# alguoo314/JASPER

Hardware: AMD Instinct MI355X
Metric: assembly Mbp/s polished + Gk-mers/s counted, k=37 (higher is better)
Workload: dtype u64

## Files before the change

### jasper_amd/csrc/polish.hip

```cpp
#include "polish.hpp"
#include <algorithm>

namespace jk {

constexpr int SMAX = 384;

__device__ __forceinline__ void pyslice(int64_t len, int64_t a, int64_t b, int64_t &lo, int64_t &hi) {
    if (a < 0) { a += len; if (a < 0) a = 0; } else if (a > len) a = len;
    if (b < 0) { b += len; if (b < 0) b = 0; } else if (b > len) b = len;
    if (b < a) b = a;
    lo = a; hi = b;
}

__device__ __forceinline__ int64_t pyround(double x) { return (int64_t)rint(x); }

struct FrontEntry {
    uint32_t node;
    uint16_t tlen;
    uint8_t alive;
    uint8_t pad;
    uint8_t tail[72];
};
static_assert(sizeof(FrontEntry) == 80, "FrontEntry layout");

// ... 951 lines not shown
                    __builtin_amdgcn_s_sleep(4);
                } else {
                    back += 64;
                    if (spins > (1u << 24)) { a = ARRIVE_FAIL; break; }
                }
            }
        }
        if (a < 0 || a < lo || a - C->seg_lo >= C->len0) {
            if (lane == 0) { C->spec_fail = 1; C->ticks = wall_clock64() - t0; }
            publish_arrival(C->arrive, ARRIVE_FAIL);
            return;
        }
        if (!dirty) {
            const int64_t stop = C->last ? C->cls_n : C->stop_orig;
            const int64_t steps = a >= stop ? 0 : (stop - a + (k - 2)) / (k - 1);
            if (lane == 0) {
                C->took_shortcut = 1;
                C->lookups = 2ull * (uint64_t)steps;
                C->ticks = wall_clock64() - t0;
            }
            publish_arrival(C->arrive, C->last ? ARRIVE_END : a + steps * (k - 1));
            return;
        }
        start_i = a - C->seg_lo;
    }
    Walker w;
    w.T = T; w.k = P.k; w.step = P.step; w.lane = threadIdx.x; w.solid = P.solid;
    w.buf = C->buf; w.len = C->len; w.gs = C->gs; w.glen = C->glen; w.cap = C->cap;
    w.C = C; w.chunk_id = C->chunk; w.nrec = 0; w.naux = 0; w.seqno = 0; w.nedit = 0; w.pass = pass;
    w.status = PS_OK; w.nlook = 0; for (int q = 0; q < 12; ++q) w.tk[q] = 0;
    w.s_tbf = s_tbf; w.s_t1 = s_t1; w.s_t2 = s_t2; w.s_gkb = s_gkb; w.s_gka = s_gka;
    w.delta = 0; w.dirty_end = INT64_MIN / 2; w.glo = P.k;
    w.is_first = C->first != 0; w.is_last = C->last != 0; w.spec_fail = 0;
    w.cls = C->cls; w.cls_n = C->cls_n; w.seg_lo = C->seg_lo; w.stop_orig = C->stop_orig;
    w.pool = pool; w.bfs_slot = -1; w.bfs_nodes = nullptr; w.bfs_front = nullptr; w.bfs_patch = nullptr;
    const bool fix = P.fix && pass < P.passes;
    int64_t wrong = 0;
    long long arrive = ARRIVE_FAIL;
    w.walk(fix, start_i, wrong, arrive);
    w.release_scratch();
    if (threadIdx.x == 0) {
        C->ticks = wall_clock64() - t0;
        for (int q = 0; q < 12; ++q) C->tk[q] = w.tk[q];
        C->len = w.len; C->gs = w.gs; C->glen = w.glen;
        C->nrec = w.nrec; C->naux = w.naux; C->nedit = w.nedit; C->status = w.status; C->spec_fail = w.spec_fail;
        C->wrong = wrong;
        C->lookups = w.nlook;
    }
    publish_arrival(C->arrive, arrive);
}

constexpr int SC_THREADS = 256, SC_GROUP = 16, SC_TILE = SC_THREADS * SC_GROUP, SC_HALO = 4;

__global__ __launch_bounds__(256) void seg_init_kernel(SegDev *segs, int n_segs, const uint8_t *const *chunk_text) {
    struct __attribute__((packed, aligned(1))) V16 { uint32_t w[4]; };
    for (int s = blockIdx.y; s < n_segs; s += gridDim.y) {
        const SegDev S = segs[s];
        const uint8_t *src = chunk_text[S.chunk] + S.seg_lo;
        uint8_t *dst = S.buf + S.glen;
        const int64_t nblk = (S.len0 + 15) >> 4;
        for (int64_t blk = blockIdx.x * (int64_t)blockDim.x + threadIdx.x; blk < nblk; blk += (int64_t)gridDim.x * blockDim.x) {
            const int64_t q0 = blk << 4;
            if (q0 + 16 <= S.len0) *reinterpret_cast<V16 *>(dst + q0) = *reinterpret_cast<const V16 *>(src + q0);
            else for (int64_t q = q0; q < S.len0; ++q) dst[q] = src[q];
        }
    }
}

constexpr uint32_t STITCH_MAX_EDITS = 32;
__global__ __launch_bounds__(256) void seg_stitch_kernel(const SegDev *segs, int n_segs, uint8_t *const *chunk_out, uint8_t *const *cls_out,
                                                         uint8_t *const *flags) {
    struct __attribute__((packed, aligned(1))) V16 { uint32_t w[4]; };
    for (int s = blockIdx.y; s < n_segs; s += gridDim.y) {
        const SegDev S = segs[s];
        uint8_t *dst = chunk_out[S.chunk] + S.out_off;
        uint8_t *cdst = cls_out ? cls_out[S.chunk] + S.out_off : nullptr;
        uint8_t *fl = cls_out ? flags[S.chunk] : nullptr;
        const int64_t n = S.own_hi - S.own_lo;
        const bool all_dirty = S.nedit > STITCH_MAX_EDITS;
        const int64_t nblk = (n + 15) >> 4;
        for (int64_t blk = blockIdx.x * (int64_t)blockDim.x + threadIdx.x; blk < nblk; blk += (int64_t)gridDim.x * blockDim.x) {
            const int64_t q0 = blk << 4;
            const int64_t p0 = S.own_lo + q0;
            const bool full = q0 + 16 <= n;
            bool text_done = false, cls_done = !cdst;
            if (full && (p0 + 16 <= S.gs || p0 >= S.gs)) {
                *reinterpret_cast<V16 *>(dst + q0) = *reinterpret_cast<const V16 *>(S.buf + (p0 < S.gs ? p0 : p0 + S.glen));
                text_done = true;
            }
            if (full && cdst && !all_dirty) {
                int64_t lA = p0, lB = p0 + 15;
                bool uniform = true;
                for (int e = (int)S.nedit - 1; e >= 0; --e) {
                    const EditRec E = S.edits[e];
                    if (lA > E.a + E.plen) { const int64_t d = (int64_t)E.plen - E.oldlen; lA -= d; lB -= d; }
                    else if (lB < E.a - 1) { }
                    else { uniform = false; break; }
                }
                if (uniform && S.seg_lo + lB < S.cls_n) {
                    *reinterpret_cast<V16 *>(cdst + q0) = *reinterpret_cast<const V16 *>(S.cls + S.seg_lo + lA);
                    cls_done = true;
                }
            }
            if (text_done && cls_done) continue;
            const int64_t qe = q0 + 16 < n ? q0 + 16 : n;
            for (int64_t q = q0; q < qe; ++q) {
                const int64_t p = S.own_lo + q;
                if (!text_done) dst[q] = S.buf[p < S.gs ? p : p + S.glen];
                if (cls_done) continue;
                int64_t l = p;
                bool dirty = all_dirty;
                if (!dirty)
                    for (int e = (int)S.nedit - 1; e >= 0; --e) {
                        const EditRec E = S.edits[e];
                        if (l > E.a + E.plen) l -= (int64_t)E.plen - E.oldlen;
                        else if (l >= E.a - 1) { dirty = true; break; }
                    }
                if (dirty) {
                    fl[(S.out_off + q) >> 6] = 1;
                    cdst[q] = PC_OTHER;
                } else {
                    const int64_t old = S.seg_lo + l;
                    cdst[q] = old < S.cls_n ? S.cls[old] : (uint8_t)PC_OTHER;
                }
            }
        }
    }
}

__global__ __launch_bounds__(64) void seg_gather_kernel(const SegDev *segs, int n_segs, const int64_t *idx_base, const uint32_t *seq_base,
                                                        const uint32_t *rec_off, const uint32_t *aux_off, FixRec *out_recs, uint8_t *out_aux) {
    const int s = blockIdx.x;
    if (s >= n_segs) return;
    const SegDev S = segs[s];
    for (uint32_t r = threadIdx.x; r < S.nrec; r += blockDim.x) {
        FixRec f = S.recs[r];
        f.index += idx_base[s];
        f.seqno += seq_base[s];
        if (f.kind == 'x') f.aux_off += aux_off[s];
        out_recs[rec_off[s] + r] = f;
    }
    for (uint32_t q = threadIdx.x; q < S.naux; q += blockDim.x) out_aux[aux_off[s] + q] = S.aux[q];
}

__device__ __forceinline__ long long wave_scan_incl64(long long v) {
    const int lane = threadIdx.x & 63;
#pragma unroll
    for (int o = 1; o < 64; o <<= 1) { const long long u = __shfl_up(v, o); if (lane >= o) v += u; }
    return v;
}
__global__ __launch_bounds__(64) void seg_summary_kernel(SegDev *segs, const int32_t *first_seg, int n_chunks, int64_t *idx_base, uint32_t *seq_base,
                                                         uint32_t *rec_off, uint32_t *aux_off, ChunkSummary *out) {
    const int c = blockIdx.x;
    if (c >= n_chunks) return;
    const int lane = threadIdx.x;
    const int s0 = first_seg[c], s1 = first_seg[c + 1];
    long long newlen = 0, shift = 0, seqc = 0, recc = 0, auxc = 0, wrong = 0, lookups = 0;
    int bad = -1, spec = 0;
    for (int base = s0; base < s1; base += 64) {
        const int s = base + lane;
        const bool in = s < s1;
        long long d = 0, own = 0, nrec = 0, naux = 0, seg_lo = 0, own_hi = 0;
        if (in) {
            SegDev &S = segs[s];
            d = S.len - S.len0;
            own_hi = S.last ? S.len : S.own_hi0 + d;
            own = own_hi - S.own_lo;
            nrec = S.nrec; naux = S.naux; seg_lo = S.seg_lo;
            wrong += S.wrong; lookups += (long long)S.lookups;
            if (S.status != PS_OK && (bad < 0 || s < bad)) bad = s;
            if (S.spec_fail && S.status == PS_OK) spec = 1;
        }
        const long long i_own = wave_scan_incl64(own), i_d = wave_scan_incl64(d), i_rec = wave_scan_incl64(nrec), i_aux = wave_scan_incl64(naux);
        if (in) {
            SegDev &S = segs[s];
            S.own_hi = own_hi;
            S.out_off = newlen + i_own - own;
            idx_base[s] = seg_lo + shift + i_d - d;
            seq_base[s] = (uint32_t)(seqc + i_rec - nrec);
            rec_off[s] = (uint32_t)(recc + i_rec - nrec);
            aux_off[s] = (uint32_t)(auxc + i_aux - naux);
        }
        newlen += __shfl(i_own, 63); shift += __shfl(i_d, 63);
        seqc += __shfl(i_rec, 63); recc += __shfl(i_rec, 63); auxc += __shfl(i_aux, 63);
    }
    for (int o = 32; o > 0; o >>= 1) {
        wrong += __shfl_xor(wrong, o); lookups += __shfl_xor(lookups, o);
        const int b2 = __shfl_xor(bad, o);
        bad = bad < 0 ? b2 : (b2 < 0 ? bad : (b2 < bad ? b2 : bad));
        spec |= __shfl_xor(spec, o);
    }
    if (lane == 0) {
        ChunkSummary R;
        R.newlen = newlen; R.wrong = wrong; R.lookups = (uint64_t)lookups; R.nrec = (uint32_t)recc; R.naux = (uint32_t)auxc; R.bad_seg = bad; R.spec_fail = spec;
        out[c] = R;
    }
}
__global__ __launch_bounds__(64) void seg_offsets_kernel(const int32_t *first_seg, int n_chunks, uint32_t *rec_off, uint32_t *aux_off, const ChunkSummary *sum) {
    const int c = blockIdx.x;
    if (c >= n_chunks || c == 0) return;
    const int lane = threadIdx.x;
    unsigned long long rb = 0, ab = 0;
    for (int q = lane; q < c; q += 64) { rb += sum[q].nrec; ab += sum[q].naux; }
    for (int o = 32; o > 0; o >>= 1) { rb += __shfl_xor(rb, o); ab += __shfl_xor(ab, o); }
    for (int s = first_seg[c] + lane; s < first_seg[c + 1]; s += 64) { rec_off[s] += (uint32_t)rb; aux_off[s] += (uint32_t)ab; }
}

constexpr int SC_BACK = 64;
constexpr int SC_STRIDE = SC_TILE - SC_BACK;
__global__ __launch_bounds__(SC_THREADS) void scan_classify_batch_kernel(const ScanChunk *__restrict__ chunks, int n_chunks, TableDev T, uint32_t solid) {
    __shared__ uint32_t s_code[SC_THREADS + SC_HALO];
    __shared__ uint32_t s_inv[SC_THREADS + SC_HALO];
    __shared__ uint32_t s_cnt[SC_TILE];
    __shared__ uint8_t s_ok[SC_TILE];
    const int t = threadIdx.x;
    const int k = T.k;
    const u128 kmask = maskbits(2 * k);
    for (int ci = blockIdx.y; ci < n_chunks; ci += gridDim.y) {
        const ScanChunk C = chunks[ci];
        const uint8_t *__restrict__ text = C.text;
        const int64_t n = C.len;
        const int64_t nwin = n - k + 1;
        if (nwin <= 0) continue;
        const int64_t ntiles = (n + SC_STRIDE - 1) / SC_STRIDE;
        for (int64_t tile = blockIdx.x; tile < ntiles; tile += gridDim.x) {
            const int64_t origin = tile * SC_STRIDE - SC_BACK;
            uint32_t c, iv;
            stage16(text, origin + (int64_t)t * SC_GROUP, n, c, iv);
            s_code[t + SC_HALO] = c;
            s_inv[t + SC_HALO] = iv;
            if (t < SC_HALO) {
                uint32_t hc, hiv;
                stage16(text, origin - (int64_t)(SC_HALO - t) * SC_GROUP, n, hc, hiv);
                s_code[t] = hc;
                s_inv[t] = hiv;
            }
            __syncthreads();
            const uint32_t w4 = s_code[t], w3 = s_code[t + 1], w2 = s_code[t + 2], w1 = s_code[t + 3];
            const uint64_t ivprev = ((uint64_t)s_inv[t] << 48) | ((uint64_t)s_inv[t + 1] << 32) | ((uint64_t)s_inv[t + 2] << 16) |
                                    (uint64_t)s_inv[t + 3];
            u128 fwd = band(mk(((uint64_t)w4 << 32) | w3, ((uint64_t)w2 << 32) | w1), kmask);
            u128 rc = revcomp(fwd, k);
            int run = ivprev ? (int)__builtin_ctzll(ivprev) : 64;
            const int64_t e0 = origin + (int64_t)t * SC_GROUP;
#pragma unroll
            for (int j0 = 0; j0 < SC_GROUP; j0 += 4) {
                u128 hs[4];
                bool ok[4];
                ulonglong2 ent[4];
#pragma unroll
                for (int u = 0; u < 4; ++u) {
                    const int j = j0 + u;
                    const uint32_t cj = (c >> (30 - 2 * j)) & 3u;
                    const bool bad = (iv >> (15 - j)) & 1u;
                    fwd = band(bor(shl(fwd, 2), mk(0, cj)), kmask);
                    rc = bor(shr(rc, 2), shl(mk(0, 3u - cj), 2 * (k - 1)));
                    run = bad ? 0 : run + 1;
                    const int64_t e = e0 + j;
                    ok[u] = run >= k && e - k + 1 >= 0 && e < n;
                    hs[u] = mix(lt(rc, fwd) ? rc : fwd, T.B);
                    ent[u] = make_ulonglong2(0ull, 0ull);
                    if (ok[u]) ent[u] = *reinterpret_cast<const ulonglong2 *>(read_slots(T, hs[u]) + 2 * home_of(hs[u], T.B, T.s));
                }
#pragma unroll
                for (int u = 0; u < 4; ++u) {
                    s_cnt[t * SC_GROUP + j0 + u] = ok[u] ? clamp32(table_get_prefetched(T, hs[u], ent[u])) : 0u;
                    s_ok[t * SC_GROUP + j0 + u] = ok[u] ? 1 : 0;
                }
            }
            __syncthreads();
            if (t >= SC_BACK / SC_GROUP) {
                struct __attribute__((packed, aligned(1))) V16 { uint32_t w[4]; };
                V16 out;
                out.w[0] = out.w[1] = out.w[2] = out.w[3] = 0;
                const int64_t p0 = e0 - k + 1;
#pragma unroll
                for (int j = 0; j < SC_GROUP; ++j) {
                    const int64_t p = p0 + j;
                    const uint32_t me = s_cnt[t * SC_GROUP + j];
                    uint8_t cl;
                    if (!s_ok[t * SC_GROUP + j]) cl = PC_OTHER;
                    else if (me < solid) cl = PC_BAD;
                    else if (p > 0) {
                        const int64_t qe = (p - k > 0 ? p - k : 0) + k - 1;
                        const int qi = (int)(qe - origin);
                        cl = (!s_ok[qi] || 50ull * me < (unsigned long long)s_cnt[qi]) ? PC_OTHER : PC_CLEAN;
                    } else cl = PC_CLEAN;
                    out.w[j >> 2] |= (uint32_t)cl << (8 * (j & 3));
                }
                if (p0 >= 0 && p0 + SC_GROUP <= nwin) *reinterpret_cast<V16 *>(C.cls + p0) = out;
                else {
#pragma unroll
                    for (int j = 0; j < SC_GROUP; ++j) {
                        const int64_t p = p0 + j;
                        if (p >= 0 && p < nwin) C.cls[p] = (uint8_t)((out.w[j >> 2] >> (8 * (j & 3))) & 0xFFu);
                    }
                }
            }
            __syncthreads();
        }
    }
}

__global__ __launch_bounds__(256) void find_sync_batch_kernel(const ScanChunk *__restrict__ chunks, int n_chunks, int k) {
    struct __attribute__((packed, aligned(1))) V16 { uint32_t w[4]; };
    const int64_t W = 4ll * k;
    for (int ci = blockIdx.y; ci < n_chunks; ci += gridDim.y) {
        const ScanChunk C = chunks[ci];
        if (!C.want_sync) continue;
        const int64_t nwin = C.len - k + 1;
        const uint8_t *__restrict__ cls = C.cls;
        static_assert(PC_CLEAN == 0 && PC_BAD == 1 && PC_OTHER == 2, "the block test below looks at bit 0 of the class bytes");
        const int64_t nblk = (nwin + 15) >> 4;
        for (int64_t blk = blockIdx.x * (int64_t)blockDim.x + threadIdx.x; blk < nblk; blk += (int64_t)gridDim.x * blockDim.x) {
            const int64_t p0 = blk << 4;
            uint32_t w[4];
            if (p0 + 16 <= nwin) {
                const V16 v = *reinterpret_cast<const V16 *>(cls + p0);
                w[0] = v.w[0]; w[1] = v.w[1]; w[2] = v.w[2]; w[3] = v.w[3];
                if (!((w[0] | w[1] | w[2] | w[3]) & 0x01010101u)) continue;
            }
            const int64_t pe = p0 + 16 < nwin ? p0 + 16 : nwin;
            for (int64_t p = p0; p < pe; ++p) {
                if (p < W || p + k - 1 > nwin) continue;
                if (cls[p] != PC_BAD || cls[p - 1] != PC_CLEAN) continue;
                uint32_t diff = 0;
                {
                    int64_t q = p + 1;
                    const int64_t qe = p + k - 1;
                    for (; q + 16 <= qe; q += 16) {
                        const V16 v = *reinterpret_cast<const V16 *>(cls + q);
                        diff |= (v.w[0] ^ 0x01010101u) | (v.w[1] ^ 0x01010101u) | (v.w[2] ^ 0x01010101u) | (v.w[3] ^ 0x01010101u);
                    }
                    for (; q < qe; ++q) diff |= (uint32_t)(cls[q] ^ (uint8_t)PC_BAD);
                    q = p - W;
                    const int64_t qf = p - 1;
                    for (; q + 16 <= qf; q += 16) {
                        const V16 v = *reinterpret_cast<const V16 *>(cls + q);
                        diff |= v.w[0] | v.w[1] | v.w[2] | v.w[3];
                    }
                    for (; q < qf; ++q) diff |= (uint32_t)cls[q];
                }
                if (diff) continue;
                const unsigned int idx = atomicAdd(C.cand_count, 1u);
                if (idx < C.cand_cap) C.cand[idx] = ((int64_t)ci << 40) | p;
            }
        }
    }
}

__global__ __launch_bounds__(256) void rescan_batch_kernel(const ScanChunk *__restrict__ chunks, int n_chunks, TableDev T, uint32_t solid) {
    __shared__ uint32_t s_cnt[4][128];
    __shared__ uint8_t s_valid[4][128];
    __shared__ uint8_t s_text[4][256];
    const int wave = threadIdx.x >> 6, lane = threadIdx.x & 63;
    const int k = T.k;
    for (int ci = blockIdx.y; ci < n_chunks; ci += gridDim.y) {
        const ScanChunk C = chunks[ci];
        const int64_t nwin = C.len - k + 1;
        if (nwin <= 0) continue;
        const int64_t ntile = (nwin + 63) >> 6, nflag = (C.len >> 6) + 1;
        const int64_t W = (int64_t)gridDim.x * 4;
        for (int64_t tile0 = (int64_t)blockIdx.x * 4 + wave; tile0 < ntile; tile0 += 64 * W) {
            uint8_t f = 0;
            {
                const int64_t tl = tile0 + (int64_t)lane * W;
                if (tl < ntile) {
                    f = C.flags[tl];
                    if (tl > 0) f |= C.flags[tl - 1];
                    if (tl + 1 < nflag) f |= C.flags[tl + 1];
                }
            }
            unsigned long long todo = __ballot(f != 0);
          while (todo) {
            const int64_t tile = tile0 + (int64_t)__builtin_ctzll(todo) * W;
            todo &= todo - 1ull;
            const int64_t base = tile * 64 - 64;
#pragma unroll
            for (int q = 0; q < 4; ++q) {
                const int64_t pos = base + (int64_t)lane * 4 + q;
                s_text[wave][lane * 4 + q] = (pos >= 0 && pos < C.len) ? C.text[pos] : (uint8_t)'N';
            }
            __builtin_amdgcn_fence(__ATOMIC_SEQ_CST, "workgroup");
            __builtin_amdgcn_wave_barrier();
#pragma unroll
            for (int r = 0; r < 2; ++r) {
                const int64_t p = base + r * 64 + lane;
                uint32_t cnt = 0;
                uint8_t valid = 0;
                if (p >= 0 && p < nwin) {
                    u128 fwd = mk(0, 0);
                    bool ok = true;
                    for (int j = 0; j < k; ++j) {
                        const int c = code(s_text[wave][r * 64 + lane + j]);
                        ok = ok && c >= 0;
                        fwd = bor(shl(fwd, 2), mk(0, (uint64_t)(c & 3)));
                    }
                    if (ok) {
                        cnt = clamp32(table_get(T, mix(canonical(fwd, k), T.B)));
                        valid = 1;
                    }
                }
                s_cnt[wave][r * 64 + lane] = cnt;
                s_valid[wave][r * 64 + lane] = valid;
            }
            __builtin_amdgcn_fence(__ATOMIC_SEQ_CST, "workgroup");
            __builtin_amdgcn_wave_barrier();
            const int64_t p = tile * 64 + lane;
            if (p < nwin) {
                const int me = 64 + lane;
                uint8_t c;
                if (!s_valid[wave][me]) c = PC_OTHER;
                else if (s_cnt[wave][me] < solid) c = PC_BAD;
                else if (p > 0) {
                    const int qi = p - k > 0 ? me - k : 64;
                    c = (!s_valid[wave][qi] || 50ull * s_cnt[wave][me] < (unsigned long long)s_cnt[wave][qi]) ? PC_OTHER : PC_CLEAN;
                } else c = PC_CLEAN;
                C.cls[p] = c;
            }
            __builtin_amdgcn_wave_barrier();
          }
        }
    }
}

__global__ __launch_bounds__(64) void find_clean_batch_kernel(const ScanChunk *__restrict__ chunks, int n_chunks, int k) {
    const int lane = threadIdx.x;
    for (int ci = blockIdx.y; ci < n_chunks; ci += gridDim.y) {
        const ScanChunk C = chunks[ci];
        const int64_t nwin = C.len - k + 1;
        for (uint32_t g = blockIdx.x; g < C.n_cells; g += gridDim.x) {
            int64_t p0 = (int64_t)g * CLEAN_CELL + CLEAN_CELL / 2;
            const int64_t cell_end = (int64_t)(g + 1) * CLEAN_CELL;
            int64_t cand = -1;
            for (int attempt = 0; attempt < 8; ++attempt) {
                if (p0 - 4ll * k < 0 || p0 + k > nwin || p0 + k > cell_end) break;
                int64_t last_bad = -1;
                for (int64_t q0 = p0 - 4ll * k; q0 < p0 + k; q0 += 64) {
                    const int64_t q = q0 + lane;
                    const bool nc = q < p0 + k && C.cls[q] != PC_CLEAN;
                    const uint64_t m = __ballot(nc);
                    if (m) last_bad = q0 + 63 - (int64_t)__builtin_clzll(m);
                }
                if (last_bad < 0) { cand = p0; break; }
                p0 = last_bad + 4ll * k + 1;
            }
            if (lane == 0) C.clean_cand[g] = cand;
        }
    }
}

static void launch_find_clean(const ScanChunk *d_chunks, int n_chunks, int k, hipStream_t stream) {
    const int gy = n_chunks < 1024 ? n_chunks : 1024;
    const int gx = std::max(1, 8192 / gy);
    hipLaunchKernelGGL(find_clean_batch_kernel, dim3(gx, gy), dim3(64), 0, stream, d_chunks, n_chunks, k);
}

void launch_rescan_batch(const TableDev &T, const ScanChunk *d_chunks, int n_chunks, int k, uint32_t solid, hipStream_t stream) {
    if (n_chunks <= 0) return;
    const int gy = n_chunks < 1024 ? n_chunks : 1024;
    const int gx = std::max(1, 4096 / gy);
    hipLaunchKernelGGL(rescan_batch_kernel, dim3(gx, gy), dim3(256), 0, stream, d_chunks, n_chunks, T, solid);
    hipLaunchKernelGGL(find_sync_batch_kernel, dim3(gx, gy), dim3(256), 0, stream, d_chunks, n_chunks, k);
    launch_find_clean(d_chunks, n_chunks, k, stream);
}

void launch_scan_batch(const TableDev &T, const ScanChunk *d_chunks, int n_chunks, int k, uint32_t solid, hipStream_t stream) {
    if (n_chunks <= 0) return;
    const int gy = n_chunks < 1024 ? n_chunks : 1024;
    const int gx = std::max(1, 4096 / gy);
    hipLaunchKernelGGL(scan_classify_batch_kernel, dim3(gx, gy), dim3(SC_THREADS), 0, stream, d_chunks, n_chunks, T, solid);
    hipLaunchKernelGGL(find_sync_batch_kernel, dim3(gx, gy), dim3(256), 0, stream, d_chunks, n_chunks, k);
    launch_find_clean(d_chunks, n_chunks, k, stream);
}

__global__ __launch_bounds__(256) void copy_chunks_kernel(uint8_t *const *__restrict__ chunk_ptr, uint8_t *__restrict__ pack, const int64_t *__restrict__ offs, int n,
                                                          int to_chunks) {
    for (int c = blockIdx.x; c < n; c += gridDim.x) {
        const int64_t len = offs[c + 1] - offs[c];
        uint8_t *a = chunk_ptr[c], *b = pack + offs[c];
        const uint8_t *src = to_chunks ? b : a;
        uint8_t *dst = to_chunks ? a : b;
        for (int64_t i = threadIdx.x; i < len; i += 256) dst[i] = src[i];
    }
}
void launch_copy_chunks(uint8_t *const *d_chunk_ptr, uint8_t *d_pack, const int64_t *d_offs, int n, bool to_chunks, hipStream_t stream) {
    if (n <= 0) return;
    hipLaunchKernelGGL(copy_chunks_kernel, dim3((unsigned)std::min(n, 256 * 16)), dim3(256), 0, stream, d_chunk_ptr, d_pack, d_offs, n, to_chunks ? 1 : 0);
}

void launch_seg_init(SegDev *d_segs, int n_segs, const uint8_t *const *d_chunk_text, hipStream_t stream) {
    if (n_segs <= 0) return;
    dim3 grid(n_segs >= 512 ? 4 : 64, n_segs < 4096 ? n_segs : 4096);
    hipLaunchKernelGGL(seg_init_kernel, grid, dim3(256), 0, stream, d_segs, n_segs, d_chunk_text);
}
void launch_seg_walk(const TableDev &T, SegDev *d_segs, int n_segs, PolishParams pp, int pass, ScratchPool pool, unsigned int *d_ticket,
                     hipStream_t stream) {
    if (n_segs <= 0) return;
    (void)hipMemsetAsync(d_ticket, 0, sizeof(unsigned int), stream);
    hipLaunchKernelGGL(seg_walk_kernel, dim3(n_segs), dim3(64), 0, stream, T, d_segs, n_segs, pp, pass, pool, d_ticket);
}
void launch_seg_summary(SegDev *d_segs, int n_segs, const int32_t *d_first_seg, int n_chunks, int64_t *idx_base, uint32_t *seq_base, uint32_t *rec_off,
                        uint32_t *aux_off, ChunkSummary *d_out, hipStream_t stream) {
    if (n_segs <= 0 || n_chunks <= 0) return;
    hipLaunchKernelGGL(seg_summary_kernel, dim3(n_chunks), dim3(64), 0, stream, d_segs, d_first_seg, n_chunks, idx_base, seq_base, rec_off, aux_off, d_out);
    hipLaunchKernelGGL(seg_offsets_kernel, dim3(n_chunks), dim3(64), 0, stream, d_first_seg, n_chunks, rec_off, aux_off, d_out);
}
void launch_seg_gather(const SegDev *d_segs, int n_segs, const int64_t *idx_base, const uint32_t *seq_base, const uint32_t *rec_off,
                       const uint32_t *aux_off, FixRec *out_recs, uint8_t *out_aux, hipStream_t stream) {
    if (n_segs <= 0) return;
    hipLaunchKernelGGL(seg_gather_kernel, dim3(n_segs), dim3(64), 0, stream, d_segs, n_segs, idx_base, seq_base, rec_off, aux_off, out_recs, out_aux);
}
void launch_seg_stitch(const SegDev *d_segs, int n_segs, uint8_t *const *d_chunk_out, uint8_t *const *d_cls_out, uint8_t *const *d_flags,
                       hipStream_t stream) {
    if (n_segs <= 0) return;
    dim3 grid(n_segs >= 2048 ? 2 : n_segs >= 512 ? 4 : 64, n_segs < 4096 ? n_segs : 4096);
    hipLaunchKernelGGL(seg_stitch_kernel, grid, dim3(256), 0, stream, d_segs, n_segs, d_chunk_out, d_cls_out, d_flags);
}

}
```

Measured before the change: 3057.

## Add specialized dense-table rescan kernel and fuse sync/clean mark kernels

```diff
diff --git a/jasper_amd/csrc/polish.hip b/jasper_amd/csrc/polish.hip
--- a/jasper_amd/csrc/polish.hip
+++ b/jasper_amd/csrc/polish.hip
@@ -1277,12 +1277,113 @@
     }
 }
 
-__global__ __launch_bounds__(256) void find_sync_batch_kernel(const ScanChunk *__restrict__ chunks, int n_chunks, int k) {
+template <int NW, int KFIX>
+struct DenseCore {
+    int k, sh;
+    int rsh;
+    uint32_t topmask, slotmask;
+    uint64_t lomask, himask, remmask;
+    uint32_t f[NW], r[NW];
+    __device__ __forceinline__ explicit DenseCore(const TableDev &T) {
+        k = KFIX ? KFIX : T.k;
+        const int B = 2 * k, topbits = B - 32 * (NW - 1), hb = B - 64;
+        sh = B - T.s;
+        rsh = topbits - 2;
+        topmask = topbits >= 32 ? ~0u : ((1u << topbits) - 1u);
+        slotmask = (uint32_t)T.mask;
+        lomask = B >= 64 ? ~0ull : ((1ull << B) - 1ull);
+        himask = NW > 2 ? (hb >= 64 ? ~0ull : ((1ull << hb) - 1ull)) : 0ull;
+        remmask = (1ull << sh) - 1ull;
+    }
+    __device__ __forceinline__ void start(u128 fwd0, u128 rc0) {
+        const uint32_t fw[4] = {(uint32_t)fwd0.lo, (uint32_t)(fwd0.lo >> 32), (uint32_t)fwd0.hi, (uint32_t)(fwd0.hi >> 32)};
+        const uint32_t rw[4] = {(uint32_t)rc0.lo, (uint32_t)(rc0.lo >> 32), (uint32_t)rc0.hi, (uint32_t)(rc0.hi >> 32)};
+#pragma unroll
+        for (int w = 0; w < NW; ++w) { f[w] = fw[w]; r[w] = rw[w]; }
+    }
+    __device__ __forceinline__ void roll(uint32_t cj) {
+#pragma unroll
+        for (int w = NW - 1; w > 0; --w) f[w] = __builtin_amdgcn_alignbit(f[w], f[w - 1], 30);
+        f[0] = (f[0] << 2) | cj;
+        f[NW - 1] &= topmask;
+#pragma unroll
+        for (int w = 0; w < NW - 1; ++w) r[w] = __builtin_amdgcn_alignbit(r[w + 1], r[w], 2);
+        r[NW - 1] = (r[NW - 1] >> 2) | ((cj ^ 3u) << rsh);
+    }
+    __device__ __forceinline__ void probe(uint32_t &home, uint64_t &want0) const {
+        static_assert(NW >= 1 && NW <= 3, "a narrow table holds no k-mer of more than three words: 2k - s <= 53");
+        uint32_t m[NW];
+        [[maybe_unused]] uint32_t d;
+        if constexpr (NW == 3) {
+            asm("v_sub_co_u32_e32 %3, vcc, %4, %7\n\tv_subb_co_u32_e32 %3, vcc, %5, %8, vcc\n\tv_subb_co_u32_e32 %3, vcc, %6, %9, vcc\n\t"
+                "v_cndmask_b32_e32 %0, %7, %4, vcc\n\tv_cndmask_b32_e32 %1, %8, %5, vcc\n\tv_cndmask_b32_e32 %2, %9, %6, vcc"
+                : "=&v"(m[0]), "=&v"(m[1]), "=&v"(m[2]), "=&v"(d) : "v"(r[0]), "v"(r[1]), "v"(r[2]), "v"(f[0]), "v"(f[1]), "v"(f[2]) : "vcc");
+        } else if constexpr (NW == 2) {
+            asm("v_sub_co_u32_e32 %2, vcc, %3, %5\n\tv_subb_co_u32_e32 %2, vcc, %4, %6, vcc\n\t"
+                "v_cndmask_b32_e32 %0, %5, %3, vcc\n\tv_cndmask_b32_e32 %1, %6, %4, vcc"
+                : "=&v"(m[0]), "=&v"(m[1]), "=&v"(d) : "v"(r[0]), "v"(r[1]), "v"(f[0]), "v"(f[1]) : "vcc");
+        } else {
+            m[0] = r[0] < f[0] ? r[0] : f[0];
+        }
+        uint64_t rem;
+        if constexpr (NW > 2) {
+            const uint64_t lo = mix64(((uint64_t)m[1] << 32) | m[0]);
+            const uint64_t hi = ((uint64_t)m[2] ^ rotr64(lo, 30)) & himask;
+            home = (uint32_t)((lo >> sh) | (hi << (64 - sh)));
+            rem = lo & remmask;
+        } else {
+            const int hh = k;
+            uint64_t v = m[0];
+            if constexpr (NW > 1) v |= (uint64_t)m[1] << 32;
+            v ^= v >> hh;
+            v = (v * JK_C1) & lomask;
+            v ^= v >> hh;
+            home = (uint32_t)(v >> sh);
+            rem = v & remmask;
+        }
+        want0 = OCC | (rem << OFFBITS);
+    }
+};
+static bool dense_core_serves(const TableDev &T) { return !T.ext && T.nshard <= 1 && T.s <= 32 && 2 * T.k - T.s >= 0 && 2 * T.k - T.s <= 63 - OFFBITS; }
+
+__device__ __forceinline__ ulonglong2 dense_load(const TableDev &T, uint32_t slotmask, uint32_t home, uint32_t off) {
+    return *reinterpret_cast<const ulonglong2 *>(T.slots + 2ull * (uint64_t)((home + off) & slotmask));
+}
+template <int U0, int U1, int N>
+__device__ __forceinline__ void dense_resolve(const ulonglong2 (&ent)[N], const uint64_t (&want0)[N], uint32_t off, uint32_t (&cnt)[N], uint32_t &pend) {
+#pragma unroll
+    for (int u = U0; u < U1; ++u) {
+        if ((pend >> u) & 1u) {
+            const bool hit = ent[u].x == want0[u] + off;
+            if (hit) cnt[u] = clamp32(ent[u].y);
+            if (hit || ent[u].x == 0ull) pend &= ~(1u << u);
+        }
+    }
+}
+template <int U0, int U1, int N>
+__device__ __forceinline__ void dense_issue(const TableDev &T, uint32_t slotmask, const uint32_t (&home)[N], uint32_t off, uint32_t pend, ulonglong2 (&ent)[N]) {
+#pragma unroll
+    for (int u = U0; u < U1; ++u)
+        if ((pend >> u) & 1u) ent[u] = dense_load(T, slotmask, home[u], off);
+}
+template <int N>
+__device__ __forceinline__ void dense_counts(const TableDev &T, uint32_t slotmask, const uint32_t (&home)[N], const uint64_t (&want0)[N], ulonglong2 (&ent)[N],
+                                             uint32_t pend, uint32_t (&cnt)[N]) {
+    constexpr int H = N / 2;
+#pragma unroll
+    for (int u = 0; u < N; ++u) cnt[u] = 0;
+    dense_resolve<0, H>(ent, want0, 0, cnt, pend);
+    dense_resolve<H, N>(ent, want0, 0, cnt, pend);
+    for (uint32_t off = 1; __ballot(pend != 0) && off < MAXPROBE; ++off) {
+        dense_issue<0, N>(T, slotmask, home, off, pend, ent);
+        dense_resolve<0, N>(ent, want0, off, cnt, pend);
+    }
+}
+
+__device__ __forceinline__ void find_sync_chunk(const ScanChunk &C, int ci, int k) {
     struct __attribute__((packed, aligned(1))) V16 { uint32_t w[4]; };
     const int64_t W = 4ll * k;
-    for (int ci = blockIdx.y; ci < n_chunks; ci += gridDim.y) {
-        const ScanChunk C = chunks[ci];
-        if (!C.want_sync) continue;
+    {
         const int64_t nwin = C.len - k + 1;
         const uint8_t *__restrict__ cls = C.cls;
         static_assert(PC_CLEAN == 0 && PC_BAD == 1 && PC_OTHER == 2, "the block test below looks at bit 0 of the class bytes");
@@ -1295,10 +1396,24 @@
                 w[0] = v.w[0]; w[1] = v.w[1]; w[2] = v.w[2]; w[3] = v.w[3];
                 if (!((w[0] | w[1] | w[2] | w[3]) & 0x01010101u)) continue;
             }
-            const int64_t pe = p0 + 16 < nwin ? p0 + 16 : nwin;
-            for (int64_t p = p0; p < pe; ++p) {
+            uint32_t startm = 0;
+            if (p0 + 16 <= nwin) {
+                uint32_t badm = 0, cleanm = 0;
+#pragma unroll
+                for (int j = 0; j < 16; ++j) {
+                    const uint32_t b = (w[j >> 2] >> (8 * (j & 3))) & 0xFFu;
+                    badm |= (b == PC_BAD ? 1u : 0u) << j;
+                    cleanm |= (b == PC_CLEAN ? 1u : 0u) << j;
+                }
+                startm = badm & ((cleanm << 1) | ((p0 > 0 && cls[p0 - 1] == PC_CLEAN) ? 1u : 0u));
+            } else {
+                for (int64_t p = p0 > 0 ? p0 : 1; p < nwin; ++p)
+                    if (cls[p] == PC_BAD && cls[p - 1] == PC_CLEAN) startm |= 1u << (int)(p - p0);
+            }
+            while (startm) {
+                const int64_t p = p0 + __builtin_ctz(startm);
+                startm &= startm - 1u;
                 if (p < W || p + k - 1 > nwin) continue;
-                if (cls[p] != PC_BAD || cls[p - 1] != PC_CLEAN) continue;
                 uint32_t diff = 0;
                 {
                     int64_t q = p + 1;
@@ -1399,12 +1514,98 @@
     }
 }
 
-__global__ __launch_bounds__(64) void find_clean_batch_kernel(const ScanChunk *__restrict__ chunks, int n_chunks, int k) {
-    const int lane = threadIdx.x;
+template <int NW, int KFIX>
+__global__ __launch_bounds__(256) void rescan_core_kernel(const ScanChunk *__restrict__ chunks, int n_chunks, TableDev T, uint32_t solid) {
+    constexpr int PADW = 4, TEXTW = 12;
+    __shared__ uint32_t s_cnt[4][128];
+    __shared__ uint8_t s_valid[4][128];
+    __shared__ uint32_t s_cw[4][PADW + TEXTW], s_iw[4][PADW + TEXTW];
+    const int wave = threadIdx.x >> 6, lane = threadIdx.x & 63;
+    DenseCore<NW, KFIX> K(T);
+    const int k = K.k;
+    const u128 kmask = maskbits(2 * k);
+    const uint64_t kbits = k >= 64 ? ~0ull : ((1ull << k) - 1ull);
+    if (lane < PADW) { s_cw[wave][lane] = 0; s_iw[wave][lane] = 0; }
     for (int ci = blockIdx.y; ci < n_chunks; ci += gridDim.y) {
         const ScanChunk C = chunks[ci];
         const int64_t nwin = C.len - k + 1;
-        for (uint32_t g = blockIdx.x; g < C.n_cells; g += gridDim.x) {
+        if (nwin <= 0) continue;
+        const int64_t ntile = (nwin + 63) >> 6, nflag = (C.len >> 6) + 1;
+        const int64_t W = (int64_t)gridDim.x * 4;
+        for (int64_t tile0 = (int64_t)blockIdx.x * 4 + wave; tile0 < ntile; tile0 += 64 * W) {
+            uint8_t f = 0;
+            {
+                const int64_t tl = tile0 + (int64_t)lane * W;
+                if (tl < ntile) {
+                    f = C.flags[tl];
+                    if (tl > 0) f |= C.flags[tl - 1];
+                    if (tl + 1 < nflag) f |= C.flags[tl + 1];
+                }
+            }
+            unsigned long long todo = __ballot(f != 0);
+          while (todo) {
+            const int64_t tile = tile0 + (int64_t)__builtin_ctzll(todo) * W;
+            todo &= todo - 1ull;
+            const int64_t base = tile * 64 - 64;
+            if (lane < TEXTW) {
+                uint32_t c, iv;
+                stage16(C.text, base + (int64_t)lane * 16, C.len, c, iv);
+                s_cw[wave][PADW + lane] = c;
+                s_iw[wave][PADW + lane] = iv;
+            }
+            __builtin_amdgcn_fence(__ATOMIC_SEQ_CST, "workgroup");
+            __builtin_amdgcn_wave_barrier();
+            uint32_t home[2], cnt[2], want = 0;
+            uint64_t want0[2];
+            ulonglong2 ent[2];
+            {
+                const int q = 2 * lane + k, wi = q >> 4, sb = q & 15;
+                const uint32_t *cw = s_cw[wave] + wi, *iw = s_iw[wave] + wi;
+                const u128 hi4 = mk(((uint64_t)cw[0] << 32) | cw[1], ((uint64_t)cw[2] << 32) | cw[3]);
+                const u128 fwd0 = band(bor(shl(hi4, 2 * sb), mk(0, sb ? (uint64_t)(cw[4] >> (32 - 2 * sb)) : 0ull)), kmask);
+                uint64_t inv = ((((uint64_t)iw[0] << 48) | ((uint64_t)iw[1] << 32) | ((uint64_t)iw[2] << 16) | (uint64_t)iw[3]) << sb) | (uint64_t)(iw[4] >> (16 - sb));
+                K.start(fwd0, revcomp(fwd0, k));
+                const int64_t p = base + 2 * lane;
+                if (!(inv & kbits) && p >= 0 && p < nwin) want |= 1u;
+                K.probe(home[0], want0[0]);
+                ent[0] = dense_load(T, K.slotmask, home[0], 0);
+                const uint32_t cq = s_cw[wave][PADW + wi], iq = s_iw[wave][PADW + wi];
+                K.roll((cq >> (30 - 2 * sb)) & 3u);
+                inv = (inv << 1) | (uint64_t)((iq >> (15 - sb)) & 1u);
+                if (!(inv & kbits) && p + 1 >= 0 && p + 1 < nwin) want |= 2u;
+                K.probe(home[1], want0[1]);
+                ent[1] = dense_load(T, K.slotmask, home[1], 0);
+            }
+            dense_counts<2>(T, K.slotmask, home, want0, ent, want, cnt);
+            s_cnt[wave][2 * lane] = cnt[0];
+            s_cnt[wave][2 * lane + 1] = cnt[1];
+            s_valid[wave][2 * lane] = (uint8_t)(want & 1u);
+            s_valid[wave][2 * lane + 1] = (uint8_t)((want >> 1) & 1u);
+            __builtin_amdgcn_fence(__ATOMIC_SEQ_CST, "workgroup");
+            __builtin_amdgcn_wave_barrier();
+            const int64_t p = tile * 64 + lane;
+            if (p < nwin) {
+                const int me = 64 + lane;
+                uint8_t c;
+                if (!s_valid[wave][me]) c = PC_OTHER;
+                else if (s_cnt[wave][me] < solid) c = PC_BAD;
+                else if (p > 0) {
+                    const int qi = p - k > 0 ? me - k : 64;
+                    c = (!s_valid[wave][qi] || 50ull * s_cnt[wave][me] < (unsigned long long)s_cnt[wave][qi]) ? PC_OTHER : PC_CLEAN;
+                } else c = PC_CLEAN;
+                C.cls[p] = c;
+            }
+            __builtin_amdgcn_wave_barrier();
+          }
+        }
+    }
+}
+
+__device__ __forceinline__ void find_clean_chunk(const ScanChunk &C, int k, uint32_t wave_id, uint32_t n_waves) {
+    const int lane = threadIdx.x & 63;
+    {
+        const int64_t nwin = C.len - k + 1;
+        for (uint32_t g = wave_id; g < C.n_cells; g += n_waves) {
             int64_t p0 = (int64_t)g * CLEAN_CELL + CLEAN_CELL / 2;
             const int64_t cell_end = (int64_t)(g + 1) * CLEAN_CELL;
             int64_t cand = -1;
@@ -1424,20 +1625,26 @@
         }
     }
 }
-
-static void launch_find_clean(const ScanChunk *d_chunks, int n_chunks, int k, hipStream_t stream) {
-    const int gy = n_chunks < 1024 ? n_chunks : 1024;
-    const int gx = std::max(1, 8192 / gy);
-    hipLaunchKernelGGL(find_clean_batch_kernel, dim3(gx, gy), dim3(64), 0, stream, d_chunks, n_chunks, k);
+__global__ __launch_bounds__(256) void find_marks_batch_kernel(const ScanChunk *__restrict__ chunks, int n_chunks, int k) {
+    for (int ci = blockIdx.y; ci < n_chunks; ci += gridDim.y) {
+        const ScanChunk C = chunks[ci];
+        if (C.want_sync) find_sync_chunk(C, ci, k);
+        find_clean_chunk(C, k, blockIdx.x * 4u + (threadIdx.x >> 6), gridDim.x * 4u);
+    }
 }
 
 void launch_rescan_batch(const TableDev &T, const ScanChunk *d_chunks, int n_chunks, int k, uint32_t solid, hipStream_t stream) {
     if (n_chunks <= 0) return;
     const int gy = n_chunks < 1024 ? n_chunks : 1024;
     const int gx = std::max(1, 4096 / gy);
-    hipLaunchKernelGGL(rescan_batch_kernel, dim3(gx, gy), dim3(256), 0, stream, d_chunks, n_chunks, T, solid);
-    hipLaunchKernelGGL(find_sync_batch_kernel, dim3(gx, gy), dim3(256), 0, stream, d_chunks, n_chunks, k);
-    launch_find_clean(d_chunks, n_chunks, k, stream);
+    const dim3 grid(gx, gy), block(256);
+    const int nw = (2 * k + 31) / 32;
+    if (!dense_core_serves(T) || getenv("JASPER_EXPERIMENT_NO_DENSE_CORE")) hipLaunchKernelGGL(rescan_batch_kernel, grid, block, 0, stream, d_chunks, n_chunks, T, solid);
+    else if (k == 37) hipLaunchKernelGGL((rescan_core_kernel<3, 37>), grid, block, 0, stream, d_chunks, n_chunks, T, solid);
+    else if (nw == 1) hipLaunchKernelGGL((rescan_core_kernel<1, 0>), grid, block, 0, stream, d_chunks, n_chunks, T, solid);
+    else if (nw == 2) hipLaunchKernelGGL((rescan_core_kernel<2, 0>), grid, block, 0, stream, d_chunks, n_chunks, T, solid);
+    else hipLaunchKernelGGL((rescan_core_kernel<3, 0>), grid, block, 0, stream, d_chunks, n_chunks, T, solid);
+    hipLaunchKernelGGL(find_marks_batch_kernel, grid, block, 0, stream, d_chunks, n_chunks, k);
 }
 
 void launch_scan_batch(const TableDev &T, const ScanChunk *d_chunks, int n_chunks, int k, uint32_t solid, hipStream_t stream) {
@@ -1445,8 +1652,7 @@
     const int gy = n_chunks < 1024 ? n_chunks : 1024;
     const int gx = std::max(1, 4096 / gy);
     hipLaunchKernelGGL(scan_classify_batch_kernel, dim3(gx, gy), dim3(SC_THREADS), 0, stream, d_chunks, n_chunks, T, solid);
-    hipLaunchKernelGGL(find_sync_batch_kernel, dim3(gx, gy), dim3(256), 0, stream, d_chunks, n_chunks, k);
-    launch_find_clean(d_chunks, n_chunks, k, stream);
+    hipLaunchKernelGGL(find_marks_batch_kernel, dim3(gx, gy), dim3(256), 0, stream, d_chunks, n_chunks, k);
 }
 
 __global__ __launch_bounds__(256) void copy_chunks_kernel(uint8_t *const *__restrict__ chunk_ptr, uint8_t *__restrict__ pack, const int64_t *__restrict__ offs, int n,
```

Result: faster. 3089, median of 6 (+1.0%).
